# cychomatica/AudioPure

Measured on AMD Instinct MI355X. Metric: purified 1s@16kHz utterances/sec at 5 reverse steps, higher is better.
Workload: dtype f32

## Files before the change

audiopure_amd/csrc/ap_resblock_f32w.hip:

```cpp
#include "ap_common.h"

#include <type_traits>

namespace ap {

namespace {

constexpr int WC_ = 256;
constexpr int NP_ = 32;
constexpr int KCW_ = 32;
constexpr int NCH_ = WC_ / KCW_;
constexpr int XS_ = KCW_ + 4;
constexpr int XCOMP_ = NP_ * XS_;
constexpr int XBUF_ = 4 * XCOMP_;
constexpr int GS_ = WC_ + 4;
constexpr int GOFF_ = 2 * XBUF_;
constexpr int POFF_ = GOFF_ + 64 * GS_;
constexpr int PS_ = 36;
constexpr int LDS_FLOATS_ = GOFF_ + 64 * GS_;
constexpr int LDS_FLOATS_Q16_ = POFF_ + 4 * 2 * 32 * PS_;
constexpr int NCONST_ = 5 * WC_;
constexpr int DIET_CARRY_ = 2;
constexpr int DIET_CONST_ = 4;
constexpr int DIET_ROWS_ = 16;
constexpr int DIET_PK_ = 32;
constexpr int DIET_ZERO_ = 128;
#ifndef AP_F32W_DIET
#define AP_F32W_DIET 182
#endif
constexpr int DIET4_ = 0;
constexpr unsigned UNIT_BYTES_ = 4 * 64 * 16;
constexpr unsigned W1W_WAVE_BYTES_ = NCH_ * 4 * 4 * UNIT_BYTES_;
constexpr unsigned W2W_WAVE_BYTES_ = (WC_ / 8) * UNIT_BYTES_;

}

__global__ void pack_w1w_kernel(const float *__restrict__ w1f, float *__restrict__ out) {
  constexpr int C = WC_;
  const unsigned idx = blockIdx.x * blockDim.x + threadIdx.x;
  if (idx >= 4u * NCH_ * 4 * 4 * 4 * 64 * 4) return;
  const int e = idx & 3, lane = (idx >> 2) & 63, rt = (idx >> 8) & 3, comp = (idx >> 10) & 3, kg = (idx >> 12) & 3,
            ch = (idx >> 14) & 7, w = idx >> 17;
  const int i = lane & 31, hh = lane >> 5;
  const int c = 32 * ch + 8 * kg + 4 * hh + e;
  const int o = (rt & 1) * C + 64 * w + 32 * (rt >> 1) + i;
  const float *p = w1f + ((size_t)o * C + c) * 3;
  const double w0 = p[0], w1 = p[1], w2 = p[2];
  const double v = comp == 0 ? w0 : comp == 1 ? (w0 + w1 + w2) * 0.5 : comp == 2 ? (w0 - w1 + w2) * 0.5 : w2;
  out[idx] = (float)v;
}

__global__ void pack_w2w_kernel(const float *__restrict__ w2f, float *__restrict__ out) {
  constexpr int C = WC_;
  const unsigned idx = blockIdx.x * blockDim.x + threadIdx.x;
  if (idx >= 4u * (C / 8) * 4 * 64 * 4) return;
  const int e = idx & 3, lane = (idx >> 2) & 63, rt = (idx >> 8) & 3, kg = (idx >> 10) & 31, w = idx >> 15;
  const int i = lane & 31, hh = lane >> 5;
  const int c = 8 * kg + 4 * hh + e;
  const int o = (rt >> 1) * C + 64 * w + 32 * (rt & 1) + i;
  out[idx] = w2f[(size_t)o * C + c];
}

int launch_pack_f32w(ap_ctx *ctx, hipStream_t st) {
  const int C = ctx->C, S = ctx->S;
  const size_t n1f = (size_t)2 * C * C * 3, n2 = (size_t)(C + S) * C, n1w = (size_t)4 * 2 * C * C;
  for (int n = 0; n < ctx->NL; n++) {
    pack_w1w_kernel<<<(unsigned)((n1w + 255) / 256), 256, 0, st>>>(ctx->w1f + n * n1f, ctx->w1w + n * n1w);
    pack_w2w_kernel<<<(unsigned)((n2 + 255) / 256), 256, 0, st>>>(ctx->w2f + n * n2, ctx->w2w + n * n2);
  }
  AP_HIP(hipGetLastError());
  return 0;
}

template <bool NOH, bool SAVE = false, bool Q16 = false, int DIET = AP_F32W_DIET>
__global__ __launch_bounds__(256, 1) void resblock_f32w_kernel(
    const float *__restrict__ hin, const float *__restrict__ pt, float *__restrict__ hout, float *__restrict__ skip,
    const float *__restrict__ w1w, const float *__restrict__ b1, const float *__restrict__ w2w,
    const float *__restrict__ b2, int L, int logd, int accumulate, int ntiles, int nblk, float *__restrict__ aout) {
  constexpr int C = WC_;
  constexpr bool CARRY = (DIET & DIET_CARRY_) != 0, CONST = (DIET & DIET_CONST_) != 0;
  constexpr bool ROWS = Q16 && !NOH && (DIET & DIET_ROWS_) != 0;
  constexpr bool PK = Q16 && (DIET & DIET_PK_) != 0;
  constexpr bool ZERO = Q16 && (DIET & DIET_ZERO_) != 0;
  constexpr int COFF_ = Q16 ? LDS_FLOATS_Q16_ : LDS_FLOATS_;
  __shared__ __attribute__((aligned(16))) float lds[COFF_ + (CONST ? NCONST_ : 0)];

  const int tid = threadIdx.x;
  const int lane = tid & 63;
  const int wave = __builtin_amdgcn_readfirstlane(tid >> 6);
  const int j = lane & 31, hh = lane >> 5;
  const int sq = tid >> 5;
  const int d = 1 << logd;

  int t_first, t_step, t_end;
  {
    const int g = blockIdx.x, G = gridDim.x;
    if (G >= 8 && (G & 7) == 0) {
      const int xcd = g & 7, idx = g >> 3, q = nblk >> 3, r = nblk & 7;
      const int base = xcd < r ? xcd * (q + 1) : r * (q + 1) + (xcd - r) * q;
      t_first = base + idx;
      t_step = G >> 3;
      t_end = base + q + (xcd < r ? 1 : 0);
    } else {
      t_first = g;
      t_step = G;
      t_end = nblk;
    }
  }
  if (t_first >= t_end) return;
  if constexpr (CONST) {
    for (int i = tid; i < NCONST_; i += 256) lds[COFF_ + i] = i < 2 * C ? b1[i] : i < 4 * C ? b2[i - 2 * C] : pt[i - 4 * C];
    __syncthreads();
  }

  auto uni_rsrc = [&](const void *base, unsigned bytes) {
    const uint64_t hb = (uint64_t)base;
    const uint32_t lo = __builtin_amdgcn_readfirstlane((uint32_t)hb);
    const uint32_t hi = __builtin_amdgcn_readfirstlane((uint32_t)(hb >> 32));
    return __builtin_amdgcn_make_buffer_rsrc((void *)(((uint64_t)hi << 32) | lo), 0, (int)bytes, 0x00020000);
  };
  const unsigned clip_bytes = (unsigned)C * (unsigned)L * 4u;
  const __amdgpu_buffer_rsrc_t w1rs = uni_rsrc(reinterpret_cast<const char *>(w1w) + (size_t)wave * W1W_WAVE_BYTES_, W1W_WAVE_BYTES_);
  const __amdgpu_buffer_rsrc_t w2rs = uni_rsrc(reinterpret_cast<const char *>(w2w) + (size_t)wave * W2W_WAVE_BYTES_, W2W_WAVE_BYTES_);
  const unsigned lane16 = (unsigned)lane * 16u;
  const __amdgpu_buffer_rsrc_t b1rs = uni_rsrc(b1, 2u * C * 4u), b2rs = uni_rsrc(b2, 2u * C * 4u), ptrs = uni_rsrc(pt, C * 4u);
  auto ld4 = [&](const __amdgpu_buffer_rsrc_t &rs, int idx) {
    return __builtin_bit_cast(f32x4, __builtin_amdgcn_raw_buffer_load_b128(rs, (unsigned)idx * 4u, 0, 0));
  };
  int cbase = COFF_ + 64 * wave + 4 * hh;
  if constexpr (CONST && ROWS) asm volatile("" : "+v"(cbase));
  auto ld_c = [&](int idx) {
    if constexpr (ROWS) return *reinterpret_cast<const f32x4 *>(lds + cbase + (idx - 64 * wave - 4 * hh));
    else return *reinterpret_cast<const f32x4 *>(lds + COFF_ + idx);
  };
  auto ld_b1 = [&](int idx) { if constexpr (CONST) return ld_c(idx); else return ld4(b1rs, idx); };
  auto ld_b2 = [&](int idx) { if constexpr (CONST) return ld_c(2 * C + idx); else return ld4(b2rs, idx); };
  auto ld_pt = [&](int idx) { if constexpr (CONST) return ld_c(4 * C + idx); else return ld4(ptrs, idx); };

  auto load_a1 = [&](f32x4(&a)[4], unsigned unit) {
#pragma unroll
    for (int rt = 0; rt < 4; rt++)
      a[rt] = __builtin_bit_cast(f32x4, __builtin_amdgcn_raw_buffer_load_b128(w1rs, lane16 + rt * 1024u, unit * UNIT_BYTES_, 0));
  };
  auto load_a2 = [&](f32x4(&a)[4], unsigned kg) {
#pragma unroll
    for (int rt = 0; rt < 4; rt++)
      a[rt] = __builtin_bit_cast(f32x4, __builtin_amdgcn_raw_buffer_load_b128(w2rs, lane16 + rt * 1024u, kg * UNIT_BYTES_, 0));
  };

  const int col0 = d >= 32 ? j : (((j >> logd) << (logd + 1)) + (j & (d - 1)));
  const int col1 = d >= 32 ? 32 + j : col0 + d;

  int b, p0;
  __amdgpu_buffer_rsrc_t hrs;
  unsigned voff[4];
  bool tok[4];
  auto set_tile = [&](int tile) {
    b = __builtin_amdgcn_readfirstlane(tile / ntiles);
    p0 = __builtin_amdgcn_readfirstlane((tile % ntiles) * NP_);
    hrs = uni_rsrc(hin + (size_t)b * C * L, clip_bytes);
    const int p = p0 + j;
    const int tf = ((p >> logd) << (logd + 1)) + (p & (d - 1));
#pragma unroll
    for (int k = 0; k < 4; k++) {
      const int tp = tf + (k - 1) * d;
      tok[k] = (tp >= 0) && (tp < L);
      voff[k] = ((unsigned)min(max(tp, 0), L - 1) + (unsigned)(4 * sq) * (unsigned)L) * 4u;
    }
  };
    float xr[4][4];
    f32x4 ptq;
    auto issue_x = [&](int ch) {
      ptq = __builtin_bit_cast(f32x4, __builtin_amdgcn_raw_buffer_load_b128(ptrs, (unsigned)(16 * sq), ch * KCW_ * 4, 0));
#pragma unroll
      for (int cc = 0; cc < 4; cc++)
#pragma unroll
        for (int k = 0; k < 4; k++)
          xr[cc][k] = __builtin_bit_cast(float, __builtin_amdgcn_raw_buffer_load_b32(hrs, voff[k], (ch * KCW_ + cc) * L * 4, 0));
    };
    auto store_x = [&](float *dst) {
      asm volatile("" : "+v"(xr[0][0]), "+v"(xr[0][1]), "+v"(xr[0][2]), "+v"(xr[0][3]), "+v"(xr[1][0]), "+v"(xr[1][1]), "+v"(xr[1][2]),
                   "+v"(xr[1][3]), "+v"(xr[2][0]), "+v"(xr[2][1]), "+v"(xr[2][2]), "+v"(xr[2][3]), "+v"(xr[3][0]), "+v"(xr[3][1]),
                   "+v"(xr[3][2]), "+v"(xr[3][3]), "+v"(ptq));
      f32x4 c0, c1, c2, c3;
#pragma unroll
      for (int cc = 0; cc < 4; cc++) {
        const float u0 = tok[0] ? xr[cc][0] + ptq[cc] : 0.f;
        const float u1 = tok[1] ? xr[cc][1] + ptq[cc] : 0.f;
        const float u2 = tok[2] ? xr[cc][2] + ptq[cc] : 0.f;
        const float u3 = tok[3] ? xr[cc][3] + ptq[cc] : 0.f;
        c0[cc] = u0 - u2;
        c1[cc] = u1 + u2;
        c2[cc] = u2 - u1;
        c3[cc] = u3 - u1;
      }
      float *q = dst + j * XS_ + 4 * sq;
      *reinterpret_cast<f32x4 *>(q) = c0;
      *reinterpret_cast<f32x4 *>(q + XCOMP_) = c1;
      *reinterpret_cast<f32x4 *>(q + 2 * XCOMP_) = c2;
      *reinterpret_cast<f32x4 *>(q + 3 * XCOMP_) = c3;
    };

    f32x4 a[4][4];
    set_tile(t_first);
#pragma unroll
    for (int u = 0; u < 4; u++) load_a1(a[u], (unsigned)u);
    issue_x(0);

#pragma unroll 1
  for (int tile = t_first; tile < t_end; tile += t_step) {
    f32x16 acc[4][4];
#pragma unroll
    for (int rt = 0; rt < 4; rt++) {
      const int obase = (rt & 1) * C + 64 * wave + 32 * (rt >> 1);
#pragma unroll
      for (int q = 0; q < 4; q++) {
        const f32x4 bv = ld_b1(obase + 8 * q + 4 * hh);
        acc[1][rt][4 * q + 0] = bv[0];
        acc[1][rt][4 * q + 1] = bv[1];
        acc[1][rt][4 * q + 2] = bv[2];
        acc[1][rt][4 * q + 3] = bv[3];
      }
      if constexpr (!ZERO) {
#pragma unroll
        for (int r = 0; r < 16; r++) acc[0][rt][r] = acc[2][rt][r] = acc[3][rt][r] = 0.f;
      }
    }
    store_x(lds);
    __syncthreads();

    constexpr int NSTAGE = CARRY ? NCH_ - 1 : NCH_;
    const float *xfrag = lds + j * XS_ + 4 * hh;
    auto chunk = [&](int ch, auto stage_tag, auto first_tag) __attribute__((always_inline)) {
      constexpr bool STAGE = decltype(stage_tag)::value, FIRST = decltype(first_tag)::value;
      const float *xb = xfrag + (ch & 1) * XBUF_;
      if constexpr (STAGE) issue_x(ch + 1 < NCH_ ? ch + 1 : ch);
      f32x4 bq[2];
      bq[0] = *reinterpret_cast<const f32x4 *>(xb);
      __builtin_amdgcn_sched_barrier(0);
#pragma unroll
      for (int kg = 0; kg < 4; kg++) {
#pragma unroll
        for (int comp = 0; comp < 4; comp++) {
          const int u = 4 * kg + comp;
          if (u + 1 < 16) bq[(u + 1) & 1] = *reinterpret_cast<const f32x4 *>(xb + ((u + 1) & 3) * XCOMP_ + ((u + 1) >> 2) * 8);
          if (STAGE && u == 12) store_x(lds + ((ch + 1) & 1) * XBUF_);
#pragma unroll
          for (int e = 0; e < 4; e++)
#pragma unroll
            for (int rt = 0; rt < 4; rt++) {
              if (FIRST && kg == 0 && e == 0 && comp != 1)
                acc[comp][rt] = __builtin_amdgcn_mfma_f32_32x32x2f32(a[comp][rt][e], bq[u & 1][e], f32x16{}, 0, 0, 0);
              else
                acc[comp][rt] = __builtin_amdgcn_mfma_f32_32x32x2f32(a[comp][rt][e], bq[u & 1][e], acc[comp][rt], 0, 0, 0);
            }
          if (STAGE && u == 12) {
#pragma unroll
            for (int i = 0; i < 16; i++) {
              __builtin_amdgcn_sched_group_barrier(0x008, 1, 0);
              __builtin_amdgcn_sched_group_barrier(0x002, 4, 0);
            }
            __builtin_amdgcn_sched_group_barrier(0x200, 4, 0);
          }
          __builtin_amdgcn_sched_barrier(0);
          load_a1(a[comp], (unsigned)((16 * ch + u + 4) & (16 * NCH_ - 1)));
          __builtin_amdgcn_sched_barrier(0);
        }
      }
    };
    if constexpr (ZERO) {
      chunk(0, std::true_type{}, std::true_type{});
      __syncthreads();
    }
#pragma unroll 1
    for (int ch = ZERO ? 1 : 0; ch < NSTAGE; ch++) {
      chunk(ch, std::true_type{}, std::false_type{});
      __syncthreads();
    }
#pragma unroll 1
    for (int ch = NSTAGE; ch < NCH_; ch++) {
      chunk(ch, std::false_type{}, std::false_type{});
      __syncthreads();
    }

    const int tfirst = ((p0 >> logd) << (logd + 1)) + (p0 & (d - 1));
    int tcol[2];
    tcol[0] = tfirst + j;
    tcol[1] = tfirst + (d >= 32 ? d : 32) + j;
    __amdgpu_buffer_rsrc_t ars = hrs;
    unsigned sv0 = 0, sv1 = 0;
    if constexpr (SAVE) {
      ars = uni_rsrc(aout + (size_t)b * 2 * C * L, 2u * clip_bytes);
      const int pj = p0 + j;
      const int s0 = ((pj >> logd) << (logd + 1)) + (pj & (d - 1));
      sv0 = s0 < L ? (unsigned)s0 * 4u : 0x80000000u;
      sv1 = s0 + d < L ? (unsigned)(s0 + d) * 4u : 0x80000000u;
    }
    {
      float *g0 = lds + GOFF_ + col0 * GS_ + 64 * wave + 4 * hh;
      float *g1 = lds + GOFF_ + col1 * GS_ + 64 * wave + 4 * hh;
#pragma unroll
      for (int p = 0; p < 2; p++) {
#pragma unroll
        for (int c4 = 0; c4 < 4; c4++) asm volatile("" : "+a"(acc[c4][2 * p]), "+a"(acc[c4][2 * p + 1]));
#pragma unroll
        for (int q = 0; q < 4; q++) {
          f32x4 v0, v1;
          if constexpr (PK) {
#pragma unroll
            for (int e = 0; e < 4; e += 2) {
              const int r = 4 * q + e;
              auto pr = [&](const f32x16 &t) { return f32x2{t[r], t[r + 1]}; };
              const f32x2 ta = (pr(acc[0][2 * p]) + pr(acc[1][2 * p])) + pr(acc[2][2 * p]);
              const f32x2 sa = (pr(acc[0][2 * p + 1]) + pr(acc[1][2 * p + 1])) + pr(acc[2][2 * p + 1]);
              const f32x2 tb = (pr(acc[1][2 * p]) - pr(acc[2][2 * p])) + pr(acc[3][2 * p]);
              const f32x2 sb = (pr(acc[1][2 * p + 1]) - pr(acc[2][2 * p + 1])) + pr(acc[3][2 * p + 1]);
              const f32x2 ga = gate2(ta, sa), gb = gate2(tb, sb);
              v0[e] = ga[0], v0[e + 1] = ga[1];
              v1[e] = gb[0], v1[e + 1] = gb[1];
              if constexpr (SAVE) {
                const unsigned so = ((unsigned)(64 * wave + 32 * p + 4 * hh) * (unsigned)L) * 4u;
                const u32x2 tau = __builtin_bit_cast(u32x2, ta), sau = __builtin_bit_cast(u32x2, sa);
                const u32x2 tbu = __builtin_bit_cast(u32x2, tb), sbu = __builtin_bit_cast(u32x2, sb);
#pragma unroll
                for (int i = 0; i < 2; i++) {
                  const int ro = rowoff(r + i, 0) * L * 4;
                  __builtin_amdgcn_raw_buffer_store_b32(tau[i], ars, so + sv0, ro, 0);
                  __builtin_amdgcn_raw_buffer_store_b32(sau[i], ars, so + sv0 + (unsigned)C * (unsigned)L * 4u, ro, 0);
                  __builtin_amdgcn_raw_buffer_store_b32(tbu[i], ars, so + sv1, ro, 0);
                  __builtin_amdgcn_raw_buffer_store_b32(sbu[i], ars, so + sv1 + (unsigned)C * (unsigned)L * 4u, ro, 0);
                }
              }
            }
          } else {
#pragma unroll
            for (int e = 0; e < 4; e++) {
              const int r = 4 * q + e;
              const float ta = (acc[0][2 * p][r] + acc[1][2 * p][r]) + acc[2][2 * p][r];
              const float sa = (acc[0][2 * p + 1][r] + acc[1][2 * p + 1][r]) + acc[2][2 * p + 1][r];
              const float tb = (acc[1][2 * p][r] - acc[2][2 * p][r]) + acc[3][2 * p][r];
              const float sb = (acc[1][2 * p + 1][r] - acc[2][2 * p + 1][r]) + acc[3][2 * p + 1][r];
              v0[e] = gate(ta, sa);
              v1[e] = gate(tb, sb);
              if constexpr (SAVE) {
                const unsigned so = ((unsigned)(64 * wave + 32 * p + 4 * hh) * (unsigned)L) * 4u;
                const int ro = rowoff(r, 0) * L * 4;
                __builtin_amdgcn_raw_buffer_store_b32(__builtin_bit_cast(unsigned, ta), ars, so + sv0, ro, 0);
                __builtin_amdgcn_raw_buffer_store_b32(__builtin_bit_cast(unsigned, sa), ars, so + sv0 + (unsigned)C * (unsigned)L * 4u, ro, 0);
                __builtin_amdgcn_raw_buffer_store_b32(__builtin_bit_cast(unsigned, tb), ars, so + sv1, ro, 0);
                __builtin_amdgcn_raw_buffer_store_b32(__builtin_bit_cast(unsigned, sb), ars, so + sv1 + (unsigned)C * (unsigned)L * 4u, ro, 0);
              }
            }
          }
          *reinterpret_cast<f32x4 *>(g0 + 32 * p + 8 * q) = v0;
          *reinterpret_cast<f32x4 *>(g1 + 32 * p + 8 * q) = v1;
          __builtin_amdgcn_sched_barrier(0);
        }
      }
    }

    f32x16 acc2[4][2];
    {
#pragma unroll
      for (int rt = 0; rt < 4; rt++) {
        if (NOH && rt < 2) continue;
        const int cb = 64 * wave + 32 * (rt & 1);
#pragma unroll
        for (int q = 0; q < 4; q++) {
          const int c = cb + 8 * q + 4 * hh;
          f32x4 bv = ld_b2((rt < 2 ? 0 : C) + c);
          if (rt < 2) bv += ld_pt(c);
#pragma unroll
          for (int ct = 0; ct < 2; ct++) {
            acc2[rt][ct][4 * q + 0] = bv[0];
            acc2[rt][ct][4 * q + 1] = bv[1];
            acc2[rt][ct][4 * q + 2] = bv[2];
            acc2[rt][ct][4 * q + 3] = bv[3];
          }
        }
      }
    }
    f32x4 a2[2][4];
    f32x4 a2r[4][2];
    auto load_a2r = [&](f32x4(&a)[2], unsigned soff) {
#pragma unroll
      for (int r = 0; r < 2; r++)
        a[r] = __builtin_bit_cast(f32x4, __builtin_amdgcn_raw_buffer_load_b128(w2rs, lane16 + r * 1024u, soff, 0));
    };
    if constexpr (ROWS) {
#pragma unroll
      for (int k = 0; k < 4; k++) load_a2r(a2r[k], (unsigned)k * UNIT_BYTES_);
    } else {
#pragma unroll
      for (int k = 0; k < 2; k++) load_a2(a2[k], (unsigned)k);
    }

    __builtin_amdgcn_sched_barrier(0);
    float hres[Q16 ? 1 : 2][Q16 ? 1 : 2][16];
    f32x4 hq[Q16 ? 2 : 1][Q16 ? 2 : 1][4];
    unsigned eo4[2] = {0x80000000u, 0x80000000u};
    if constexpr (Q16) {
      const int rowq = lane >> 3, cq = lane & 7;
#pragma unroll
      for (int ct = 0; ct < 2; ct++) {
        const int t = tfirst + (ct ? (d >= 32 ? d : 32) : 0) + 4 * cq;
        eo4[ct] = t < L ? ((unsigned)(64 * wave + rowq) * (unsigned)L + (unsigned)t) * 4u : 0x80000000u;
      }
      if (!NOH) {
#pragma unroll
        for (int rt = 0; rt < 2; rt++)
#pragma unroll
          for (int ct = 0; ct < 2; ct++)
#pragma unroll
            for (int p = 0; p < 4; p++)
              hq[rt][ct][p] = __builtin_bit_cast(f32x4, __builtin_amdgcn_raw_buffer_load_b128(hrs, eo4[ct], (32 * rt + 8 * p) * L * 4, 2));
      }
    }
    if (!Q16 && !NOH) {
#pragma unroll
      for (int rt = 0; rt < 2; rt++)
#pragma unroll
        for (int ct = 0; ct < 2; ct++) {
          const unsigned ev = ((unsigned)(64 * wave + 32 * rt + 4 * hh) * (unsigned)L + (unsigned)min(tcol[ct], L - 1)) * 4u;
#pragma unroll
          for (int r = 0; r < 16; r++)
            hres[rt][ct][r] = __builtin_bit_cast(float, __builtin_amdgcn_raw_buffer_load_b32(hrs, ev, rowoff(r, 0) * L * 4, 2));
        }
    }
    __syncthreads();

    typedef unsigned u32x4 __attribute__((ext_vector_type(4)));
    const float RS = 0.707106781186547524f;
    if constexpr (ROWS) {
      const __amdgpu_buffer_rsrc_t ors = uni_rsrc(hout + (size_t)b * C * L, clip_bytes);
      const __amdgpu_buffer_rsrc_t sls = uni_rsrc(skip + (size_t)b * C * L, accumulate ? clip_bytes : 0u);
      const float *gfrag = lds + GOFF_ + j * GS_ + 4 * hh;
      float *patch0 = lds + POFF_ + wave * (2 * 32 * PS_);
      const int rowq = lane >> 3, cq = lane & 7;
      f32x4 bq2[2][2];
      bq2[0][0] = *reinterpret_cast<const f32x4 *>(gfrag);
      bq2[0][1] = *reinterpret_cast<const f32x4 *>(gfrag + 32 * GS_);
      __builtin_amdgcn_sched_barrier(0);
#pragma unroll 1
      for (int kg4 = 0; kg4 < C / 8; kg4 += 4) {
#pragma unroll
        for (int k = 0; k < 4; k++) {
          const int kn = (kg4 + k + 1) & (C / 8 - 1);
          bq2[(k + 1) & 1][0] = *reinterpret_cast<const f32x4 *>(gfrag + 8 * kn);
          bq2[(k + 1) & 1][1] = *reinterpret_cast<const f32x4 *>(gfrag + 32 * GS_ + 8 * kn);
#pragma unroll
          for (int e = 0; e < 4; e++)
#pragma unroll
            for (int rt = 0; rt < 2; rt++)
#pragma unroll
              for (int ct = 0; ct < 2; ct++)
                acc2[rt][ct] = __builtin_amdgcn_mfma_f32_32x32x2f32(a2r[k][rt][e], bq2[k & 1][ct][e], acc2[rt][ct], 0, 0, 0);
          __builtin_amdgcn_sched_barrier(0);
          const int nx = kg4 + k + 4;
          load_a2r(a2r[k], nx < C / 8 ? (unsigned)nx * UNIT_BYTES_ : (unsigned)(nx - C / 8) * UNIT_BYTES_ + 2048u);
          __builtin_amdgcn_sched_barrier(0);
        }
      }
#pragma unroll
      for (int t = 0; t < 4; t++) {
        const int rt = t >> 1, ct = t & 1;
        float *patch = patch0 + (t & 1) * (32 * PS_);
        f32x4 pv[4];
#pragma unroll
        for (int k8 = 0; k8 < 8; k8++) {
          const int kg = 8 * t + k8, k = kg & 3;
          if (kg + 1 < C / 8) {
            bq2[(kg + 1) & 1][0] = *reinterpret_cast<const f32x4 *>(gfrag + 8 * (kg + 1));
            bq2[(kg + 1) & 1][1] = *reinterpret_cast<const f32x4 *>(gfrag + 32 * GS_ + 8 * (kg + 1));
          }
          if (k8 == 0) {
#pragma unroll
            for (int r = 0; r < 16; r++) patch[rowoff(r, hh) * PS_ + j] = acc2[rt][ct][r];
          }
          if (k8 == 1) {
#pragma unroll
            for (int p = 0; p < 4; p++) pv[p] = *reinterpret_cast<const f32x4 *>(patch + (rowq + 8 * p) * PS_ + 4 * cq);
          }
          if (k8 == 2) {
#pragma unroll
            for (int p = 0; p < 4; p++) {
              const f32x4 o = (hq[rt][ct][p] + pv[p]) * RS;
              __builtin_amdgcn_raw_buffer_store_b128(__builtin_bit_cast(u32x4, o), ors, eo4[ct], (32 * rt + 8 * p) * L * 4, 2);
            }
          }
#pragma unroll
          for (int e = 0; e < 4; e++)
#pragma unroll
            for (int r2 = 0; r2 < 2; r2++)
#pragma unroll
              for (int c2 = 0; c2 < 2; c2++)
                acc2[2 + r2][c2] = __builtin_amdgcn_mfma_f32_32x32x2f32(a2r[k][r2][e], bq2[kg & 1][c2][e], acc2[2 + r2][c2], 0, 0, 0);
          if (k8 == 0) {
#pragma unroll
            for (int i = 0; i < 16; i++) {
              __builtin_amdgcn_sched_group_barrier(0x008, 1, 0);
              __builtin_amdgcn_sched_group_barrier(0x002, 1, 0);
              __builtin_amdgcn_sched_group_barrier(0x200, 1, 0);
            }
          }
          if (k8 == 2) {
#pragma unroll
            for (int i = 0; i < 16; i++) {
              __builtin_amdgcn_sched_group_barrier(0x008, 1, 0);
              __builtin_amdgcn_sched_group_barrier(0x002, 2, 0);
            }
            __builtin_amdgcn_sched_group_barrier(0x040, 4, 0);
          }
          __builtin_amdgcn_sched_barrier(0);
          load_a2r(a2r[k], (unsigned)((kg + 4) & (C / 8 - 1)) * UNIT_BYTES_ + 2048u);
          if (k8 == 3) {
#pragma unroll
            for (int p = 0; p < 4; p++)
              hq[rt][ct][p] = __builtin_bit_cast(f32x4, __builtin_amdgcn_raw_buffer_load_b128(sls, eo4[ct], (32 * rt + 8 * p) * L * 4, 2));
          }
          __builtin_amdgcn_sched_barrier(0);
        }
      }
    } else {
      const float *gfrag = lds + GOFF_ + j * GS_ + 4 * hh;
#pragma unroll 1
      for (int kg4 = 0; kg4 < C / 8; kg4 += 4) {
#pragma unroll
        for (int k = 0; k < 4; k++) {
          const int kg = kg4 + k;
          f32x4 bq2[2];
          bq2[0] = *reinterpret_cast<const f32x4 *>(gfrag + 8 * kg);
          bq2[1] = *reinterpret_cast<const f32x4 *>(gfrag + 32 * GS_ + 8 * kg);
#pragma unroll
          for (int e = 0; e < 4; e++)
#pragma unroll
            for (int rt = NOH ? 2 : 0; rt < 4; rt++)
#pragma unroll
              for (int ct = 0; ct < 2; ct++)
                acc2[rt][ct] = __builtin_amdgcn_mfma_f32_32x32x2f32(a2[k & 1][rt][e], bq2[ct][e], acc2[rt][ct], 0, 0, 0);
          __builtin_amdgcn_sched_barrier(0);
          load_a2(a2[k & 1], (unsigned)((kg + 2) & (C / 8 - 1)));
          __builtin_amdgcn_sched_barrier(0);
        }
      }
    }

    const __amdgpu_buffer_rsrc_t ors = uni_rsrc((NOH ? skip : hout) + (size_t)b * C * L, clip_bytes);
    const __amdgpu_buffer_rsrc_t srs = uni_rsrc(skip + (size_t)b * C * L, clip_bytes);
    if constexpr (Q16) {
      f32x4 sk4[2][2][4];
      if constexpr (ROWS) {
      } else if (accumulate) {
#pragma unroll
        for (int rt = 0; rt < 2; rt++)
#pragma unroll
          for (int ct = 0; ct < 2; ct++)
#pragma unroll
            for (int p = 0; p < 4; p++)
              sk4[rt][ct][p] = __builtin_bit_cast(f32x4, __builtin_amdgcn_raw_buffer_load_b128(srs, eo4[ct], (32 * rt + 8 * p) * L * 4, 2));
      } else {
#pragma unroll
        for (int i = 0; i < 16; i++) (&sk4[0][0][0])[i] = f32x4{0.f, 0.f, 0.f, 0.f};
      }
      float *patch0 = lds + POFF_ + wave * (2 * 32 * PS_);
      const int rowq = lane >> 3, cq = lane & 7;
      auto leave = [&](int k, const f32x16 &tile, auto &&out4) {
        float *patch = patch0 + (k & 1) * (32 * PS_);
#pragma unroll
        for (int r = 0; r < 16; r++) patch[rowoff(r, hh) * PS_ + j] = tile[r];
#pragma unroll
        for (int p = 0; p < 4; p++) out4(p, *reinterpret_cast<const f32x4 *>(patch + (rowq + 8 * p) * PS_ + 4 * cq));
      };
      {
        if (!NOH && !ROWS) {
#pragma unroll
          for (int rt = 0; rt < 2; rt++)
#pragma unroll
            for (int ct = 0; ct < 2; ct++)
              leave(2 * rt + ct, acc2[rt][ct], [&](int p, f32x4 v) {
                const f32x4 o = (hq[rt][ct][p] + v) * RS;
                __builtin_amdgcn_raw_buffer_store_b128(__builtin_bit_cast(u32x4, o), ors, eo4[ct], (32 * rt + 8 * p) * L * 4, 2);
              });
        }
      }
      {
        set_tile(tile + t_step < t_end ? tile + t_step : tile);
        if constexpr (!CARRY) {
#pragma unroll
          for (int u = 0; u < 4; u++) load_a1(a[u], (unsigned)u);
        }
        issue_x(0);
      }
      __builtin_amdgcn_sched_barrier(0);
      {
#pragma unroll
        for (int rt = 0; rt < 2; rt++)
#pragma unroll
          for (int ct = 0; ct < 2; ct++)
            leave(2 * rt + ct, acc2[2 + rt][ct], [&](int p, f32x4 v) {
              f32x4 o;
              if constexpr (ROWS) o = hq[rt][ct][p] + v; else o = sk4[rt][ct][p] + v;
              __builtin_amdgcn_raw_buffer_store_b128(__builtin_bit_cast(u32x4, o), srs, eo4[ct], (32 * rt + 8 * p) * L * 4, 2);
            });
      }
      continue;
    }
    {
      set_tile(tile + t_step < t_end ? tile + t_step : tile);
      if constexpr (!CARRY) {
#pragma unroll
        for (int u = 0; u < 4; u++) load_a1(a[u], (unsigned)u);
      }
      issue_x(0);
    }
    __builtin_amdgcn_sched_barrier(0);

    {
      typedef unsigned u32x16 __attribute__((ext_vector_type(16)));
      const float RS = 0.707106781186547524f;
#pragma unroll
      for (int rt = NOH ? 2 : 0; rt < 4; rt++) {
#pragma unroll
        for (int ct = 0; ct < 2; ct++) {
          const int t = tcol[ct];
          const unsigned eo = t < L ? ((unsigned)(64 * wave + 32 * (rt & 1) + 4 * hh) * (unsigned)L + (unsigned)t) * 4u : 0x80000000u;
          if (rt < 2) {
#pragma unroll
            for (int r = 0; r < 16; r++)
              __builtin_amdgcn_raw_buffer_store_b32(__builtin_bit_cast(unsigned, (hres[rt & 1][ct][r] + acc2[rt][ct][r]) * RS), ors, eo,
                                                    rowoff(r, 0) * L * 4, 2);
          } else if (accumulate) {
#pragma unroll
            for (int r = 0; r < 16; r++)
              (void)__builtin_amdgcn_raw_ptr_buffer_atomic_fadd_f32(acc2[rt][ct][r], srs, (int)eo, rowoff(r, 0) * L * 4, 0);
          } else {
            const u32x16 av = __builtin_bit_cast(u32x16, acc2[rt][ct]);
#pragma unroll
            for (int r = 0; r < 16; r++)
              __builtin_amdgcn_raw_buffer_store_b32(av[r], srs, eo, rowoff(r, 0) * L * 4, 2);
          }
        }
      }
    }
  }
}

#ifdef AP_TOOLS
#define AP_F32W_AB_MASKS(X) X(0) X(2) X(4) X(6) X(22) X(54) X(150)
static int g_no_q16 = 0;
static int g_diet = AP_F32W_DIET;
#else
static constexpr int g_no_q16 = 0;
#endif

bool resblock_f32w_serves(const ap_ctx *ctx, int B, int L) {
  if (ctx->cfg.precision != AP_PREC_F32 || ctx->f32_form != 1 || ctx->C != WC_ || ctx->S != WC_ || !ctx->w1w) return false;
  if ((size_t)2 * WC_ * (size_t)L * 4 >= ((size_t)1 << 31)) return false;
  return (long long)B * ((L + 2 * NP_ - 1) / (2 * NP_) + 1) < (1ll << 31);
}

int launch_resblock_f32w(ap_ctx *ctx, int layer, const float *hin, const float *pt, float *hout, float *skip, int accumulate,
                         int B, int L, hipStream_t st, float *aout) {
  if (!resblock_f32w_serves(ctx, B, L)) return 1;
  const int g_ncu = device_cu_count();
  const int logd = layer % ctx->cfg.dilation_cycle;
  const long long d = 1ll << logd;
  const long long np = (L / (2 * d)) * d + ((L % (2 * d)) < d ? (L % (2 * d)) : d);
  const int ntiles = (int)((np + NP_ - 1) / NP_);
  const long long nblk = (long long)B * ntiles;
  if (nblk >= (1ll << 31)) return 1;
  const int C = ctx->C, S = ctx->S;
  const float *w1w = ctx->w1w + (size_t)layer * 4 * 2 * C * C;
  const float *w2w = ctx->w2w + (size_t)layer * (C + S) * C;
  const float *b1 = ctx->b1 + (size_t)layer * 2 * C;
  const float *b2 = ctx->b2 + (size_t)layer * (C + S);
  const unsigned grid = (unsigned)(nblk < g_ncu ? nblk : g_ncu);
  const bool q16 = (L & 3) == 0 && !g_no_q16;
  if (aout) {
    if (!hout) { set_error("resblock (save): needs an h' buffer"); return -22; }
    if (q16) resblock_f32w_kernel<false, true, true><<<grid, 256, 0, st>>>(hin, pt, hout, skip, w1w, b1, w2w, b2, L, logd, accumulate, ntiles, (int)nblk, aout);
    else resblock_f32w_kernel<false, true, false, DIET4_><<<grid, 256, 0, st>>>(hin, pt, hout, skip, w1w, b1, w2w, b2, L, logd, accumulate, ntiles, (int)nblk, aout);
    AP_HIP(hipGetLastError());
    return 0;
  }
#ifdef AP_TOOLS
#define AP_F32W_AB(M)                                                                                                             \
  if (hout && q16 && g_diet == M) {                                                                                               \
    resblock_f32w_kernel<false, false, true, M><<<grid, 256, 0, st>>>(hin, pt, hout, skip, w1w, b1, w2w, b2, L, logd, accumulate, \
                                                                      ntiles, (int)nblk, nullptr);                                \
    AP_HIP(hipGetLastError());                                                                                                    \
    return 0;                                                                                                                     \
  }
  AP_F32W_AB_MASKS(AP_F32W_AB)
#undef AP_F32W_AB
#endif
  if (hout && q16) resblock_f32w_kernel<false, false, true><<<grid, 256, 0, st>>>(hin, pt, hout, skip, w1w, b1, w2w, b2, L, logd, accumulate, ntiles, (int)nblk, nullptr);
  else if (hout) resblock_f32w_kernel<false, false, false, DIET4_><<<grid, 256, 0, st>>>(hin, pt, hout, skip, w1w, b1, w2w, b2, L, logd, accumulate, ntiles, (int)nblk, nullptr);
  else if (q16) resblock_f32w_kernel<true, false, true><<<grid, 256, 0, st>>>(hin, pt, hout, skip, w1w, b1, w2w, b2, L, logd, accumulate, ntiles, (int)nblk, nullptr);
  else resblock_f32w_kernel<true, false, false, DIET4_><<<grid, 256, 0, st>>>(hin, pt, hout, skip, w1w, b1, w2w, b2, L, logd, accumulate, ntiles, (int)nblk, nullptr);
  AP_HIP(hipGetLastError());
  return 0;
}

}

#ifdef AP_TOOLS
extern "C" int ap_debug_f32w_q16(int on) {
  ap::g_no_q16 = on ? 0 : 1;
  return 0;
}
extern "C" int ap_debug_resblock_f32w(ap_ctx *ctx, int layer, const float *h_in, const float *part_t_layer, float *h_out, float *skip,
                                      int accumulate, int B, int L, void *stream, float *pre_gate) {
  return ap::launch_resblock_f32w(ctx, layer, h_in, part_t_layer, h_out, skip, accumulate, B, L, (hipStream_t)stream, pre_gate);
}
extern "C" int ap_debug_f32w_diet(int mask) {
  bool known = mask == AP_F32W_DIET;
#define AP_F32W_KNOWN(M) known = known || mask == M;
  AP_F32W_AB_MASKS(AP_F32W_KNOWN)
#undef AP_F32W_KNOWN
  if (!known) return -22;
  ap::g_diet = mask;
  return 0;
}
#endif
```

Baseline: 59.62.

## Move chunk-boundary barrier inside chunk loop and prefetch next X two chunks ahead

Adds a SEAM diet bit, on by default, for the Q16 path. It moves the per-chunk __syncthreads to just before the last MFMA group of each chunk and preloads the next chunk's first B fragment across the seam. It also issues the global X load two chunks ahead, interleaved with MFMAs. The aim is to hide barrier stalls and LDS/global latency at chunk boundaries, at the cost of more register pressure and more complex scheduling constraints.

```diff
diff --git a/audiopure_amd/csrc/ap_resblock_f32w.hip b/audiopure_amd/csrc/ap_resblock_f32w.hip
--- a/audiopure_amd/csrc/ap_resblock_f32w.hip
+++ b/audiopure_amd/csrc/ap_resblock_f32w.hip
@@ -25,8 +25,9 @@
 constexpr int DIET_ROWS_ = 16;
 constexpr int DIET_PK_ = 32;
 constexpr int DIET_ZERO_ = 128;
+constexpr int DIET_SEAM_ = 1024;
 #ifndef AP_F32W_DIET
-#define AP_F32W_DIET 182
+#define AP_F32W_DIET 1206
 #endif
 constexpr int DIET4_ = 0;
 constexpr unsigned UNIT_BYTES_ = 4 * 64 * 16;
@@ -82,6 +83,8 @@
   constexpr bool ROWS = Q16 && !NOH && (DIET & DIET_ROWS_) != 0;
   constexpr bool PK = Q16 && (DIET & DIET_PK_) != 0;
   constexpr bool ZERO = Q16 && (DIET & DIET_ZERO_) != 0;
+  constexpr bool SEAM = Q16 && (DIET & DIET_SEAM_) != 0;
+  static_assert(!SEAM || (CARRY && ZERO), "DIET_SEAM_ is written for the peeled first and last chunk");
   constexpr int COFF_ = Q16 ? LDS_FLOATS_Q16_ : LDS_FLOATS_;
   __shared__ __attribute__((aligned(16))) float lds[COFF_ + (CONST ? NCONST_ : 0)];
 
@@ -210,6 +213,14 @@
 #pragma unroll 1
   for (int tile = t_first; tile < t_end; tile += t_step) {
     f32x16 acc[4][4];
+    const float *xfrag = lds + j * XS_ + 4 * hh;
+    f32x4 bqc[2];
+    if constexpr (SEAM) {
+      store_x(lds);
+      __syncthreads();
+      bqc[0] = *reinterpret_cast<const f32x4 *>(xfrag);
+      __builtin_amdgcn_sched_barrier(0);
+    }
 #pragma unroll
     for (int rt = 0; rt < 4; rt++) {
       const int obase = (rt & 1) * C + 64 * wave + 32 * (rt >> 1);
@@ -226,23 +237,32 @@
         for (int r = 0; r < 16; r++) acc[0][rt][r] = acc[2][rt][r] = acc[3][rt][r] = 0.f;
       }
     }
-    store_x(lds);
-    __syncthreads();
+    if constexpr (!SEAM) {
+      store_x(lds);
+      __syncthreads();
+    }
 
     constexpr int NSTAGE = CARRY ? NCH_ - 1 : NCH_;
-    const float *xfrag = lds + j * XS_ + 4 * hh;
     auto chunk = [&](int ch, auto stage_tag, auto first_tag) __attribute__((always_inline)) {
       constexpr bool STAGE = decltype(stage_tag)::value, FIRST = decltype(first_tag)::value;
+      constexpr bool XREQ = SEAM && STAGE;
       const float *xb = xfrag + (ch & 1) * XBUF_;
-      if constexpr (STAGE) issue_x(ch + 1 < NCH_ ? ch + 1 : ch);
-      f32x4 bq[2];
-      bq[0] = *reinterpret_cast<const f32x4 *>(xb);
+      if constexpr (STAGE && (!SEAM || FIRST)) issue_x(ch + 1 < NCH_ ? ch + 1 : ch);
+      f32x4 bql[2];
+      f32x4(&bq)[2] = SEAM ? bqc : bql;
+      if constexpr (!SEAM) bq[0] = *reinterpret_cast<const f32x4 *>(xb);
       __builtin_amdgcn_sched_barrier(0);
 #pragma unroll
       for (int kg = 0; kg < 4; kg++) {
 #pragma unroll
         for (int comp = 0; comp < 4; comp++) {
           const int u = 4 * kg + comp;
+          if (SEAM && u == 15) {
+            __syncthreads();
+            if constexpr (STAGE) bq[0] = *reinterpret_cast<const f32x4 *>(xfrag + ((ch + 1) & 1) * XBUF_);
+            __builtin_amdgcn_sched_barrier(0);
+          }
+          if (XREQ && u == 13) issue_x(ch + 2 < NCH_ ? ch + 2 : NCH_ - 1);
           if (u + 1 < 16) bq[(u + 1) & 1] = *reinterpret_cast<const f32x4 *>(xb + ((u + 1) & 3) * XCOMP_ + ((u + 1) >> 2) * 8);
           if (STAGE && u == 12) store_x(lds + ((ch + 1) & 1) * XBUF_);
 #pragma unroll
@@ -262,6 +282,13 @@
             }
             __builtin_amdgcn_sched_group_barrier(0x200, 4, 0);
           }
+          if (XREQ && u == 13) {
+#pragma unroll
+            for (int i = 0; i < 16; i++) {
+              __builtin_amdgcn_sched_group_barrier(0x008, 1, 0);
+              __builtin_amdgcn_sched_group_barrier(0x020, 1, 0);
+            }
+          }
           __builtin_amdgcn_sched_barrier(0);
           load_a1(a[comp], (unsigned)((16 * ch + u + 4) & (16 * NCH_ - 1)));
           __builtin_amdgcn_sched_barrier(0);
@@ -270,17 +297,17 @@
     };
     if constexpr (ZERO) {
       chunk(0, std::true_type{}, std::true_type{});
-      __syncthreads();
+      if constexpr (!SEAM) __syncthreads();
     }
 #pragma unroll 1
     for (int ch = ZERO ? 1 : 0; ch < NSTAGE; ch++) {
       chunk(ch, std::true_type{}, std::false_type{});
-      __syncthreads();
+      if constexpr (!SEAM) __syncthreads();
     }
 #pragma unroll 1
     for (int ch = NSTAGE; ch < NCH_; ch++) {
       chunk(ch, std::false_type{}, std::false_type{});
-      __syncthreads();
+      if constexpr (!SEAM) __syncthreads();
     }
 
     const int tfirst = ((p0 >> logd) << (logd + 1)) + (p0 & (d - 1));
@@ -646,7 +673,7 @@
 }
 
 #ifdef AP_TOOLS
-#define AP_F32W_AB_MASKS(X) X(0) X(2) X(4) X(6) X(22) X(54) X(150)
+#define AP_F32W_AB_MASKS(X) X(0) X(2) X(4) X(6) X(22) X(54) X(150) X(182)
 static int g_no_q16 = 0;
 static int g_diet = AP_F32W_DIET;
 #else
```

Result: faster. 60.28, median of 6 (+1.1%).
